# SebastienCoube/Improving-performances-of-MCMC-for-Nearest-Neighbor-Gaussian-Process-models-with-full-data-augmentat

Hardware: AMD Instinct MI355X
Metric: full-field Gibbs sweeps/sec at n=1e6, m=15; achieved HBM GB/s vs roofline (higher is better)
Workload: dtype f64

## Files before the change

### improving-performances-of-mcmc-for-nearest-neighbor-gaussian-process-models-with-full-data-augmentat_amd/csrc/capi.hip

```cpp
#include <hip/hip_runtime.h>
#include <rccl/rccl.h>

#include <algorithm>
#include <climits>
#include <cmath>
#include <cstdio>
#include <cstdlib>
#include <cstring>
#include <map>
#include <atomic>
#include <mutex>
#include <new>
#include <string>
#include <vector>

#include "../../include/nngp.h"
#include "graph_prep.h"
#include "kernels.h"
#include "rec_stream.h"

using namespace nngp;

struct ChainState {
  double* linv_d[2] = {nullptr, nullptr};
// ... 1656 lines not shown
  return NNGP_OK;
}

enum SweepPart { kPrologue = 1, kColours = 2, kEpilogue = 4, kAll = 7 };

static int enqueue_sweep_body(nngp_ctx* c, int n_sweeps, int mask, const double* z_dev, int parts = kAll) {
  const int n = c->n;
  SweepDev L = sweep_dev(c);
  FieldPtrs fp;
  for (int k = 0; k < kMaxChains; ++k) fp.p[k] = k < c->C ? c->ch[k].field_d : nullptr;
  if (parts & kPrologue) {
    HIPCHK(c, launch_field_to_slots_multi(c->st, c->n, c->slot_dpos_d, fp, c->scal_d, c->w_slot_d, c->C, mask));
    HIPCHK(c, launch_spmv_chains(c->st, c->linv_cur_d, c->nn_d, n, c->b, fp, c->scal_d, c->r_d, c->C, mask));
    if (!z_dev && c->engine == 0) HIPCHK(c, launch_normals_compact(c->st, L, mask, 0, n, c->zbuf_d));
  }
  if ((parts & kColours) && c->engine == 1) {
    TileLaunch a;
    a.n_sweeps = n_sweeps;
    a.chain_mask = mask;
    a.z_in = z_dev;
    a.variant = c->tvariant;
    if (c->tcs) {
      a.stagger = c->tstagger;
      HIPCHK(c, launch_sweep_tiles_cs(c->st, tile_dev(c), a, c->tl.max_rows, c->tl.NTK, c->tl.max_batches,
                                      c->tl.max_gslots));
    } else {
      HIPCHK(c, launch_sweep_tiles(c->st, tile_dev(c), a, c->tl.max_rows, c->tl.NTK, c->tl.max_batches,
                                    c->tl.max_gslots));
    }
    HIPCHK(c, hipMemcpyAsync(c->tmo_h, c->ctl_d + 2, sizeof(unsigned), hipMemcpyDeviceToHost, c->st));
  }
  if ((parts & kColours) && c->engine == 0) {
    const size_t zn = (size_t)n * c->C;
    for (int s = 0; s < n_sweeps; ++s) {
      for (int col = 0; col < c->lay.K; ++col) {
        ColorLaunch a;
        a.chunk0 = c->lay.color_chunk_ptr[col];
        a.nch = c->lay.color_chunk_ptr[col + 1] - a.chunk0;
        a.chain_mask = mask;
        a.sweep_local = s;
        a.z_cur = z_dev ? z_dev + (size_t)s * zn : c->zbuf_d + (size_t)(s & 1) * zn;
        a.z_next = (!z_dev && s + 1 < n_sweeps) ? c->zbuf_d + (size_t)((s + 1) & 1) * zn : nullptr;
        a.pairs = c->pairs_d + c->pair_ptr[col];
        a.npairs = c->pair_ptr[col + 1] - c->pair_ptr[col];
        a.n = n;
        HIPCHK(c, launch_sweep_color(c->st, L, a));
      }
    }
  }
  if (parts & kEpilogue)
    HIPCHK(c, launch_slots_to_field_multi(c->st, c->n, c->slot_dpos_d, fp, c->scal_d, c->w_slot_d, c->C, mask));
  return NNGP_OK;
}

static int graph_for(nngp_ctx* c, int n_sweeps, int mask, hipGraphExec_t* out, int parts = kAll) {
  const long long key = ((long long)n_sweeps << 12) | ((long long)parts << 8) | mask;
  auto it = c->graphs.find(key);
  if (it == c->graphs.end()) {
    hipGraph_t g;
    HIPCHK(c, hipStreamBeginCapture(c->st, hipStreamCaptureModeThreadLocal));
    int rc = enqueue_sweep_body(c, n_sweeps, mask, nullptr, parts);
    hipError_t e = hipStreamEndCapture(c->st, &g);
    if (rc) return rc;
    if (e != hipSuccess) return fail_hip(c, e, "hipStreamEndCapture");
    hipGraphExec_t ex;
// ... 1049 lines not shown
```

### improving-performances-of-mcmc-for-nearest-neighbor-gaussian-process-models-with-full-data-augmentat_amd/csrc/kernels.h

```cpp
#pragma once
#include <hip/hip_runtime.h>
#include <cstdint>
#include <vector>

namespace nngp {

constexpr int kWave = 64;
constexpr int kBlock = 256;
constexpr int kRedBlocks = 4096;

struct SweepScalars {
  double inv_s2;
  double inv_t2;
  double beta0;
  double dshift;
  uint64_t seed;
  uint64_t counter_base;
};

constexpr int kSweepRows = 16;
constexpr int kMaxChains = 4;

constexpr int kPkRowBits = 25;
constexpr int kPkPadRow = (1 << kPkRowBits) - 1;
// ... 155 lines not shown
  const double* const* b1;
  unsigned* ctl;
  unsigned long long* dbg;
  int K, C, T, n;
  int max_gslots;
  int probe = 0;
  int xw = 0;
};

struct TileLaunch {
  int n_sweeps;
  int chain_mask;
  const double* z_in;
  int stagger = 0;
  int variant = 0;
};

constexpr int tile_double_buffer(int C, int NT) { return C <= 2 ? 1 : 0; }
constexpr int tile_rmax(int C, int NT) { return 4096 / NT; }
constexpr int tile_rmax_cs(int NT) { return 2048 / NT; }
constexpr int tile_gmax(int NT) { return NT == 256 ? 4 : (NT == 512 ? 3 : 1); }
constexpr int kTileRanksMax = 16;
struct TileShard {
  int G = 1, Tl = 0, tile0 = 0, rank0 = 0;
  const TileDev* devs = nullptr;
  const unsigned* call = nullptr;
  double* gx[kTileRanksMax] = {};
};
hipError_t launch_sweep_tiles(hipStream_t st, const TileDev& D, const TileLaunch& a, int max_rows, int NT,
                              int max_batches, int max_gslots, const TileShard* sh = nullptr, int grid = 0,
// ... 47 lines not shown
```

### improving-performances-of-mcmc-for-nearest-neighbor-gaussian-process-models-with-full-data-augmentat_amd/csrc/tiles.hip

```cpp
#include "kernels.h"
#include "device_common.h"
#include "graph_prep.h"

namespace nngp {

constexpr uint32_t kTPad = kTilePadRow;
constexpr uint32_t kTStart = kCellStart, kTEnd = kCellEnd;
constexpr int kTExported = kSlotExported;
constexpr int kTSlots = kTileSlotsMax;
static_assert(kTileQShift == kTileRowBits && kTileQMask + 1 >= (uint32_t)kTSlots && kTileRowBits + 11 <= 30,
              "cell_pk fields: local row | slot << kTileQShift | start << 30 | end << 31");
constexpr int kTSpreadLds = 82 * 1024;


typedef unsigned int u32x4_t __attribute__((ext_vector_type(4)));
typedef unsigned int u32x2_t __attribute__((ext_vector_type(2)));

__device__ __forceinline__ uint32_t tile_lr(uint32_t pk) { return (pk & kTPad) ^ kTPad; }



__global__ void set_ptr_kernel(const double** dst, int k, const double* p) {
  if (threadIdx.x == 0) dst[k] = p;
}
// ... 121 lines not shown
}

template <int C, int NT, int RMAX>
__device__ __forceinline__ void tile_load_cells(const TileDev& D, const int4 B, TileBatchRegs<C, NT, RMAX>& b, int t) {
  b.R = B.y & 0xFFFF;
  const bool live = t < (B.y >> 16);
#pragma unroll
  for (int j = 0; j < RMAX; ++j) {
    if (j < b.R && live) {
      const long long e = B.x + (long long)j * NT + t;
      b.pk[j] = __builtin_nontemporal_load(D.cell_pk + e);
#pragma unroll
      for (int ch = 0; ch < C; ++ch) b.v[j][ch] = __builtin_nontemporal_load(D.cell_val + ch * D.n_cells + e);
    } else {
      b.pk[j] = 0u;
      if constexpr (NT == 64) {
#pragma unroll
        for (int ch = 0; ch < C; ++ch) b.v[j][ch] = 0.0;
      }
    }
  }
}

template <int C, int NT, int RMAX, int SH, int CS = C>
__device__ __forceinline__ void tile_load_batch(const TileDev& D, const int4 B, TileBatchRegs<C, NT, RMAX>& b, int t) {
  tile_load_items<C, NT, RMAX, SH, CS>(D, B, b, t);
  tile_load_cells<C, NT, RMAX>(D, B, b, t);
}

template <int C, int NT, int RMAX, int CS = C>
__device__ __forceinline__ void tile_prep_items(const TileDev& D, const TileLaunch& a, const double* sc_s,
                                                const unsigned long long* seed_s, int s,
                                                TileBatchRegs<C, NT, RMAX>& b, int t, int var = 0) {
#pragma unroll
// ... 5 lines not shown
      double z = 0.0;
      if (var & 2) z = 0.0;
      else if (a.z_in) z = a.z_in[((size_t)s * D.n + b.x0 + q) * CS + ch];
      else z = normal_loc(seed_s[2 * ch], seed_s[2 * ch + 1] + s, (uint32_t)b.loc[k]);
      const double a0 = (var & 4) ? 1.0 : b.a0[k], a1 = (var & 4) ? 0.5 : b.a1[k], wk = (var & 4) ? 0.0 : b.w[k];
      const double P = a0 * inv_s2 + (double)((var & 4) ? 1 : b.nobs[k]) * inv_t2;
      const double cR = inv_t2 * a1 + inv_s2 * (a0 * wk);
      const double rs = rsqrt_pos(P);
      b.a0[k] = cR;
      b.a1[k] = rs * rs;
      b.zs[k] = z * rs;
    }
  }
}

template <int C, int GMAX>
struct TileGhostRegs {
  int lr[GMAX], gx[GMAX];
  double gv[GMAX][C];
};

template <int C, int NT, int GMAX>
__device__ __forceinline__ void tile_load_ghosts(const TileDev& D, int gb, int g1, TileGhostRegs<C, GMAX>& g, int t) {
#pragma unroll
  for (int k = 0; k < GMAX; ++k) {
    const int e = gb + k * NT + t;
    g.lr[k] = -1;
    if (e < g1) {
      const long long raw = __builtin_nontemporal_load(reinterpret_cast<const long long*>(D.gcell) + e);
      g.lr[k] = (int)(raw & 0xFFFFFFFFll);
      g.gx[k] = (int)(raw >> 32);
#pragma unroll
      for (int ch = 0; ch < C; ++ch) g.gv[k][ch] = __builtin_nontemporal_load(D.gval + ch * D.n_gcells + e);
    }
  }
}

struct TileState;
template <int C, int GMAX>
__device__ __forceinline__ void tile_ghost_adds(TileState& S, const TileGhostRegs<C, GMAX>& gr);

struct TileState {
  double* r_s;
  double* acc_s;
  double* wsum;
  double* sc_s;
  unsigned long long* seed_s;
  double* dsh_s;
  int4* batch_s;
  int* bptr_s;
  int* gptr_s;
  int* gsp_s;
  int* bsp_s;
  double* gdw_s;
  int* wflag;
  unsigned* spin_s;
  int* pub_s;
  __amdgpu_buffer_rsrc_t gran;
  unsigned call;
  int gsl;
  unsigned* tmo;
  int G;
  bool timed_out;
  int T, t, lane, wv, K, nph, ph;
  uint32_t lrmax;
  unsigned long long tp[8], t_prev;
};

template <int C, int GMAX>
__device__ __forceinline__ void tile_ghost_adds(TileState& S, const TileGhostRegs<C, GMAX>& gr) {
  double rv[GMAX][C], dv[GMAX][C];
#pragma unroll
  for (int k = 0; k < GMAX; ++k) {
    const bool ok = gr.lr[k] >= 0;
    const int row = ok ? gr.lr[k] : 0, x = ok ? gr.gx[k] : 0;
#pragma unroll
    for (int ch = 0; ch < C; ++ch) {
      rv[k][ch] = S.r_s[row * C + ch];
      dv[k][ch] = S.gdw_s[x * C + ch];
    }
  }
#pragma unroll
  for (int k = 0; k < GMAX; ++k)
    if (gr.lr[k] >= 0)
#pragma unroll
      for (int ch = 0; ch < C; ++ch) S.r_s[gr.lr[k] * C + ch] = rv[k][ch] + gr.gv[k][ch] * dv[k][ch];
}

#define TSTAMP(S, k)                                                      \
  do {                                                                    \
    if (PROBE == 1) {                                                          \
      asm volatile("s_waitcnt vmcnt(0) lgkmcnt(0)" ::: "memory");         \
      const unsigned long long now_ = __builtin_amdgcn_s_memrealtime();   \
      if ((k) >= 0) (S).tp[(k) < 0 ? 0 : (k)] += now_ - (S).t_prev;       \
      (S).t_prev = now_;                                                  \
    }                                                                     \
  } while (0)

constexpr int kTimelinePhases = 512;
constexpr int kTimelineSlots = 16;
#define TLSTAMP(S, k)                                                                         \
// ... 4 lines not shown


template <int CTRL, int RM, bool BC, int C>
__device__ __forceinline__ void seg_scan_step(double (&v)[C], int& f) {
  double e[C];
#pragma unroll
  for (int ch = 0; ch < C; ++ch) e[ch] = dpp_f64<CTRL, RM, BC>(v[ch]);
  const int fe = __builtin_amdgcn_update_dpp(0, f, CTRL, RM, 0xF, BC);
  const double keep = f ? 0.0 : 1.0;
#pragma unroll
  for (int ch = 0; ch < C; ++ch) v[ch] = __builtin_fma(e[ch], keep, v[ch]);
  f |= fe;
}

constexpr int kOwnDrawBarriers = 3;
template <int C, int RMAX, int GRP, class TB>
__device__ __forceinline__ void tile_products(const TB& b, int R, const double* __restrict__ r_s,
                                              double* __restrict__ acc_s, uint32_t lrmax, double (&run)[C],
                                              int& cont_q, bool& seen_start) {
#pragma unroll
  for (int ch = 0; ch < C; ++ch) run[ch] = 0.0;
#pragma unroll
  for (int j0 = 0; j0 < RMAX; j0 += GRP) {
    if (j0 >= R) break;
    double rv[GRP][C];
#pragma unroll
    for (int jj = 0; jj < GRP; ++jj) {
      if (j0 + jj < RMAX) {
        const uint32_t lr = min(tile_lr(b.pk[j0 + jj]), lrmax);
#pragma unroll
        for (int ch = 0; ch < C; ++ch) rv[jj][ch] = r_s[lr * C + ch];
      }
    }
#pragma unroll
    for (int jj = 0; jj < GRP; ++jj) {
      const int j = j0 + jj;
      if (j < RMAX) {
        const uint32_t pk = b.pk[j];
        const bool st = (pk & kTStart) != 0;
        const double keep = st ? 0.0 : 1.0;
#pragma unroll
        for (int ch = 0; ch < C; ++ch) run[ch] = __builtin_fma(run[ch], keep, b.v[j][ch] * rv[jj][ch]);
        const int q = (int)((pk >> kTileQShift) & kTileQMask);
        if (pk & kTEnd) {
#pragma unroll
          for (int ch = 0; ch < C; ++ch) acc_s[q * C + ch] = run[ch];
// ... 15 lines not shown
  const int R = b.R, nit = b.ns * C;
  tile_cells_landed(b);
  double run[C];
  int cont_q = -1;
  bool seen_start = false;
#pragma unroll
  for (int ch = 0; ch < C; ++ch) run[ch] = 0.0;
#pragma unroll
  for (int j = 0; j < RMAX; ++j) {
    if (j < R) {
      const uint32_t pk = b.pk[j];
      const uint32_t lr = min(tile_lr(pk), S.lrmax);
      const bool st = (pk & kTStart) != 0;
      const double keep = st ? 0.0 : 1.0;
#pragma unroll
      for (int ch = 0; ch < C; ++ch) run[ch] = __builtin_fma(run[ch], keep, b.v[j][ch] * r_s[lr * C + ch]);
      const int q = (int)((pk >> kTileQShift) & kTileQMask);
      if (pk & kTEnd) {
#pragma unroll
        for (int ch = 0; ch < C; ++ch) acc_s[q * C + ch] = run[ch];
      }
      seen_start |= st;
      cont_q = ((pk & kTEnd) && !seen_start && cont_q < 0) ? q : cont_q;
    }
  }
  TSTAMP(S, 1);
  double v[C];
  int f = seen_start ? 1 : 0;
#pragma unroll
  for (int ch = 0; ch < C; ++ch) v[ch] = run[ch];
  seg_scan_step<0x111, 0xF, true, C>(v, f);
// ... 47 lines not shown
#pragma unroll
          for (int h = 0; h < kTileRanksMax; ++h)
            if (h < S.G && ((b.rm[k] >> h) & 1u))
              __builtin_amdgcn_raw_buffer_store_b128(
                  g, __builtin_amdgcn_make_buffer_rsrc(sh.gx[h], 0, 0x7FFFFFFF, 0x00020000), (int)(xu * 16), 0,
                  kGranAuxSys);
        }
      }
    }
  }
  __syncthreads();
  TSTAMP(S, 3);
  TLSTAMP(S, 1);
}

template <int C, int NT, int RMAX, int PROBE>
__device__ __forceinline__ void tile_own_scatter(TileState& S, const TileBatchRegs<C, NT, RMAX>& b, int R,
                                                 const double* acc_base = nullptr) {
  constexpr int GRP = RMAX < 4 ? RMAX : 4;
  double* r_s = S.r_s;
  const double* acc_s = acc_base ? acc_base : S.acc_s;
#pragma unroll
  for (int j0 = 0; j0 < RMAX; j0 += GRP) {
    if (j0 >= R) break;
    double rv[GRP][C], dv[GRP][C];
#pragma unroll
    for (int jj = 0; jj < GRP; ++jj) {
      const int j = j0 + jj;
      const uint32_t lr = tile_lr(b.pk[j]);
      const bool ok = j < R && lr != kTPad;
      const int row = ok ? (int)lr : 0, q = ok ? (int)((b.pk[j] >> kTileQShift) & kTileQMask) : 0;
#pragma unroll
      for (int ch = 0; ch < C; ++ch) {
        rv[jj][ch] = r_s[row * C + ch];
        dv[jj][ch] = acc_s[q * C + ch];
      }
    }
#pragma unroll
    for (int jj = 0; jj < GRP; ++jj) {
      const int j = j0 + jj;
      const uint32_t lr = tile_lr(b.pk[j]);
      if (j < R && lr != kTPad) {
#pragma unroll
        for (int ch = 0; ch < C; ++ch) r_s[lr * C + ch] = rv[jj][ch] + b.v[j][ch] * dv[jj][ch];
      }
    }
  }
  TSTAMP(S, 4);
}

template <int C, int NT, int RMAX>
__device__ __forceinline__ void tile_cells_landed(const TileBatchRegs<C, NT, RMAX>& b) {
#pragma unroll
  for (int j = 0; j < RMAX; ++j) {
    asm volatile("" ::"v"(b.pk[j]));
#pragma unroll
    for (int ch = 0; ch < C; ++ch) asm volatile("" ::"v"(b.v[j][ch]));
  }
}
// ... 197 lines not shown
    const int R = cur.R;
    if (bi + 1 == bend && more) tile_load_items<C, NT, RMAX, SH>(D, S.batch_s[S.bptr_s[cn]], cur, t);
    tile_own_scatter<C, NT, RMAX, PROBE>(S, cur, R);
  }
  if (more) {
    if (had_bnd) tile_load_cells<C, NT, RMAX>(D, S.batch_s[S.bptr_s[cn]], cur, t);
    else if (!had_int) tile_load_batch<C, NT, RMAX, SH>(D, S.batch_s[S.bptr_s[cn]], cur, t);
    tile_prep_items<C, NT, RMAX>(D, a, S.sc_s, S.seed_s, sn, cur, t);
  }
  __syncthreads();
  TLSTAMP(S, 3);
}

__device__ __forceinline__ void wave_lds_order() { asm volatile("s_waitcnt lgkmcnt(0)" ::: "memory"); }

template <int C, int RMAX, int PROBE, int SH>
__device__ __forceinline__ void tile_own_wl(const TileDev& D, const TileLaunch& a, const TileShard& sh, TileState& S,
                                            TileBatchRegs<C, 64, RMAX>& b, unsigned epoch, double* acc_w,
                                            bool first = false) {
  constexpr int IMAX = TileBatchRegs<C, 64, RMAX>::IMAX;
  const int lane = S.lane;
  const double* __restrict__ r_s = S.r_s;
  double* __restrict__ acc_s = acc_w;
  const int R = b.R, nit = b.ns * C;
  tile_cells_landed(b);
  double run[C];
  int cont_q = -1;
  bool seen_start = false;
  tile_products<C, RMAX, 4>(b, R, r_s, acc_s, S.lrmax, run, cont_q, seen_start);
  double v[C];
  int f = seen_start ? 1 : 0;
#pragma unroll
  for (int ch = 0; ch < C; ++ch) v[ch] = run[ch];
  seg_scan_step<0x111, 0xF, true, C>(v, f);
  seg_scan_step<0x112, 0xF, true, C>(v, f);
  seg_scan_step<0x114, 0xF, true, C>(v, f);
  seg_scan_step<0x118, 0xF, true, C>(v, f);
  seg_scan_step<0x142, 0xA, false, C>(v, f);
  seg_scan_step<0x143, 0xC, false, C>(v, f);
#pragma unroll
  for (int ch = 0; ch < C; ++ch) {
    const double up = dpp_f64<0x138, 0xF, true>(v[ch]);
    const double cp = lane ? up : 0.0;
    if (cont_q >= 0) acc_s[cont_q * C + ch] = acc_s[cont_q * C + ch] + cp;
// ... 22 lines not shown
          for (int h = 0; h < kTileRanksMax; ++h)
            if (h < S.G && ((b.rm[k] >> h) & 1u))
              __builtin_amdgcn_raw_buffer_store_b128(
                  g, __builtin_amdgcn_make_buffer_rsrc(sh.gx[h], 0, 0x7FFFFFFF, 0x00020000), (int)(xu * 16), 0,
                  kGranAuxSys);
        }
      }
    }
  }
  wave_lds_order();
  TLSTAMP(S, 1);
  if (PROBE == 2 && lane == 0 && S.ph < kTimelinePhases && S.wv < 7)
    D.dbg[((size_t)S.T * kTimelinePhases + S.ph) * kTimelineSlots + 9 + S.wv] = __builtin_amdgcn_s_memrealtime();
}

template <int C, int NT, int RMAX, int GMAX, int PROBE, int SH, int DB>
__device__ __forceinline__ void tile_phase_wl(const TileDev& D, const TileLaunch& a, const TileShard& sh,
                                              TileState& S, int ph, TileBatchRegs<C, 64, RMAX>& cur,
                                              TileBatchRegs<C, 64, RMAX>& nxt, TileGhostRegs<C, GMAX>& gr) {
  constexpr int W = NT / 64 - 1;
  const int K = S.K, t = S.t, lane = S.lane;
  const int s = ph / K, c = ph - s * K;
  const unsigned epoch = (unsigned)ph + 1;
  S.ph = ph;
  TLSTAMP(S, 0);
  const int phn = ph + 1;
  const int cn = phn % K, sn = phn / K;
  const bool has_next = phn < S.nph;
  const int bnext = S.bptr_s[cn] + S.wv;
  const bool more = has_next && bnext < S.bptr_s[cn + 1];
  const int bfirst = S.bptr_s[c] + S.wv, bend = S.bptr_s[c + 1];
  const int g0 = S.gptr_s[c], g1 = S.gptr_s[c + 1];
  double* acc_w = S.acc_s + S.wv * (kWaveSlotsMax * C);
  if (DB && more) tile_load_batch<C, 64, RMAX, SH>(D, S.batch_s[bnext], nxt, lane);
  for (int bi = bfirst; bi < bend; bi += W) {
    if (bi != bfirst) {
      tile_load_batch<C, 64, RMAX, SH>(D, S.batch_s[bi], cur, lane);
      tile_prep_items<C, 64, RMAX>(D, a, S.sc_s, S.seed_s, s, cur, lane);
    }
    tile_own_wl<C, RMAX, PROBE, SH>(D, a, sh, S, cur, epoch, acc_w, bi == bfirst);
    if (bi == bfirst && S.wv == 0 && lane == 0)
      __hip_atomic_store(S.pub_s, ph, __ATOMIC_RELAXED, __HIP_MEMORY_SCOPE_WORKGROUP);
    const int R = cur.R;
    if (bi + W >= bend) {
      if (!DB && more) tile_load_items<C, 64, RMAX, SH>(D, S.batch_s[bnext], nxt, lane);
      if (g1 > g0) tile_load_ghosts<C, NT, GMAX>(D, g0, g1, gr, t);
    }
    tile_own_scatter<C, 64, RMAX, PROBE>(S, cur, R, acc_w);
  }
  if (bfirst >= bend) {
    if (!DB && more) tile_load_items<C, 64, RMAX, SH>(D, S.batch_s[bnext], nxt, lane);
    if (g1 > g0) tile_load_ghosts<C, NT, GMAX>(D, g0, g1, gr, t);
  }
  TLSTAMP(S, 6);
  if (more) tile_prep_items<C, 64, RMAX>(D, a, S.sc_s, S.seed_s, sn, nxt, lane, PROBE == 2 ? a.variant : 0);
  if (!DB && more) tile_load_cells<C, 64, RMAX>(D, S.batch_s[bnext], nxt, lane);
  TLSTAMP(S, 4);
  __syncthreads();
  TLSTAMP(S, 2);
  for (int gb = g0; gb < g1; gb += NT * GMAX) {
    if (gb != g0) tile_load_ghosts<C, NT, GMAX>(D, gb, g1, gr, t);
    tile_ghost_adds<C, GMAX>(S, gr);
  }
  __syncthreads();
  TLSTAMP(S, 3);
}

template <int C, int NT, int RMAX, int GMAX, int PROBE, int SH>
__device__ __forceinline__ int tile_wlib_first(const TileState& S, int c) {
  const int fi = S.bptr_s[c] + S.wv, fb = S.bsp_s[c] + S.wv;
  return fi < S.bsp_s[c] ? fi : (fb < S.bptr_s[c + 1] ? fb : -1);
}

template <int C, int NT, int RMAX, int GMAX, int PROBE, int SH>
__device__ __forceinline__ void tile_phase_wlib(const TileDev& D, const TileLaunch& a, const TileShard& sh,
                                                TileState& S, int ph, TileBatchRegs<C, 64, RMAX>& cur,
                                                TileGhostRegs<C, GMAX>& gr) {
  constexpr int W = NT / 64 - 1;
  const int K = S.K, t = S.t, lane = S.lane;
  const int s = ph / K, c = ph - s * K;
  const unsigned epoch = (unsigned)ph + 1;
  S.ph = ph;
  TLSTAMP(S, 0);
  const int phn = ph + 1;
  const int cn = phn % K, sn = phn / K;
  const int nxt_b = phn < S.nph ? tile_wlib_first<C, NT, RMAX, GMAX, PROBE, SH>(S, cn) : -1;
  const int bsp = S.bsp_s[c], b1 = S.bptr_s[c + 1];
  const int ifirst = S.bptr_s[c] + S.wv, bfirst = bsp + S.wv;
  const bool hp = ph > 0;
  const int cp = hp ? (ph - 1) % K : 0;
  const int g0 = S.gptr_s[cp], g1 = hp ? S.gptr_s[cp + 1] : g0;
  double* acc_w = S.acc_s + S.wv * (kWaveSlotsMax * C);
  bool nx_items = false;
  for (int bi = ifirst; bi < bsp; bi += W) {
    if (bi != ifirst) {
      tile_load_batch<C, 64, RMAX, SH>(D, S.batch_s[bi], cur, lane);
      tile_prep_items<C, 64, RMAX>(D, a, S.sc_s, S.seed_s, s, cur, lane);
    }
    tile_own_wl<C, RMAX, PROBE, SH>(D, a, sh, S, cur, epoch, acc_w);
    const int R = cur.R;
    if (bi + W >= bsp) {
      if (bfirst < b1) {
        tile_load_items<C, 64, RMAX, SH>(D, S.batch_s[bfirst], cur, lane);
      } else if (nxt_b >= 0) {
        tile_load_items<C, 64, RMAX, SH>(D, S.batch_s[nxt_b], cur, lane);
        nx_items = true;
      }
      if (g1 > g0) tile_load_ghosts<C, NT, GMAX>(D, g0, g1, gr, t);
    }
    tile_own_scatter<C, 64, RMAX, PROBE>(S, cur, R, acc_w);
  }
  if (ifirst >= bsp) {
    if (g1 > g0) tile_load_ghosts<C, NT, GMAX>(D, g0, g1, gr, t);
  } else if (bfirst < b1) {
    tile_prep_items<C, 64, RMAX>(D, a, S.sc_s, S.seed_s, s, cur, lane);
    tile_load_cells<C, 64, RMAX>(D, S.batch_s[bfirst], cur, lane);
  }
  TLSTAMP(S, 6);
  __syncthreads();
  TLSTAMP(S, 4);
  for (int gb = g0; gb < g1; gb += NT * GMAX) {
    if (gb != g0) tile_load_ghosts<C, NT, GMAX>(D, gb, g1, gr, t);
    tile_ghost_adds<C, GMAX>(S, gr);
  }
  __syncthreads();
  TLSTAMP(S, 2);
  for (int bi = bfirst; bi < b1; bi += W) {
    if (bi != bfirst) {
      tile_load_batch<C, 64, RMAX, SH>(D, S.batch_s[bi], cur, lane);
      tile_prep_items<C, 64, RMAX>(D, a, S.sc_s, S.seed_s, s, cur, lane);
    }
    tile_own_wl<C, RMAX, PROBE, SH>(D, a, sh, S, cur, epoch, acc_w);
    const int R = cur.R;
    if (bi + W >= b1 && nxt_b >= 0) {
      tile_load_items<C, 64, RMAX, SH>(D, S.batch_s[nxt_b], cur, lane);
      nx_items = true;
    }
    tile_own_scatter<C, 64, RMAX, PROBE>(S, cur, R, acc_w);
  }
  if (nxt_b >= 0) {
    if (!nx_items) tile_load_items<C, 64, RMAX, SH>(D, S.batch_s[nxt_b], cur, lane);
    tile_prep_items<C, 64, RMAX>(D, a, S.sc_s, S.seed_s, sn, cur, lane);
    tile_load_cells<C, 64, RMAX>(D, S.batch_s[nxt_b], cur, lane);
  }
  __syncthreads();
  TLSTAMP(S, 3);
}


template <int C, int NT, int GMAX, int PROBE, int SH, int WL = 0, int LAG = 0>
__device__ __forceinline__ void tile_phase_xw(const TileDev& D, TileState& S, int ph, TileGhostRegs<C, GMAX>& gr) {
  constexpr int PB = 4;
  const int K = S.K, t = S.t, lane = S.lane;
  S.ph = ph;
  if (LAG && ph == 0) {
    __syncthreads();
    __syncthreads();
    __syncthreads();
    return;
  }
  const int phx = ph - LAG;
  const int c = phx % K;
  const unsigned epoch = (unsigned)phx + 1;
  const int bfirst = S.bptr_s[c], bend = S.bptr_s[c + 1];
  const int g0 = S.gptr_s[c], g1 = S.gptr_s[c + 1];
// ... 49 lines not shown
      }
      __builtin_amdgcn_s_sleep(1);
#pragma unroll
      for (int k = 0; k < PB; ++k)
        if ((pend >> k) & 1u) g[k] = __builtin_amdgcn_raw_buffer_load_b128(S.gran, off[k], 0, aux);
    }
  }
  if (PROBE == 2 && lane == 0 && S.ph < kTimelinePhases) {
    D.dbg[((size_t)S.T * kTimelinePhases + S.ph) * kTimelineSlots + 7] = __builtin_amdgcn_s_memrealtime();
    D.dbg[((size_t)S.T * kTimelinePhases + S.ph) * kTimelineSlots + 5] = *S.spin_s;
    *S.spin_s = 0;
  }
  __syncthreads();
  for (int gb = g0; gb < g1; gb += NT * GMAX) {
    if (gb != g0) tile_load_ghosts<C, NT, GMAX>(D, gb, g1, gr, t);
    tile_ghost_adds<C, GMAX>(S, gr);
  }
  __syncthreads();
  if (LAG && ph < S.nph) __syncthreads();
}

template <int C, int NT, int NTC, int RMAX, int GMAX, int DB, int PROBE, int SH>
__device__ __forceinline__ void tile_phase_cells(const TileDev& D, const TileLaunch& a, const TileShard& sh,
                                                 TileState& S, int ph, TileBatchRegs<C, NTC, RMAX>& cur,
                                                 TileBatchRegs<C, NTC, RMAX>& nxt, TileGhostRegs<C, GMAX>& gr) {
  const int K = S.K, t = S.t;
  const int s = ph / K, c = ph - s * K;
  const unsigned epoch = (unsigned)ph + 1;
  S.ph = ph;
  TLSTAMP(S, 0);
  const int phn = ph + 1;
// ... 28 lines not shown
  }
  TLSTAMP(S, 6);
  if (more) tile_prep_items<C, NTC, RMAX>(D, a, S.sc_s, S.seed_s, sn, nxt, t);
  if (!DB && more) tile_load_cells<C, NTC, RMAX>(D, S.batch_s[S.bptr_s[cn]], nxt, t);
  TLSTAMP(S, 4);
  __syncthreads();
  TLSTAMP(S, 2);
  for (int gb = g0; gb < g1; gb += NT * GMAX) {
    if (gb != g0) tile_load_ghosts<C, NT, GMAX>(D, gb, g1, gr, t);
    tile_ghost_adds<C, GMAX>(S, gr);
  }
  __syncthreads();
  TLSTAMP(S, 3);
}

template <int C, int NT, int RMAX, int GMAX, int DB, int PROBE, int SH, int RG, int IB, int CS, int XW = 0>
__device__ __forceinline__ void sweep_tiles_body(const TileDev& D0, TileLaunch a, const TileShard& sh) {
  static_assert(!XW || ((!RG || XW == 2) && (!IB || XW == 2) && CS == C),
                "exchange-wave tiles: joint chains; split layouts and r in global memory only with wave-local batches");
  constexpr int NTC = XW ? NT - 64 : NT;
  using BR = TileBatchRegs<C, NTC, RMAX>;
  constexpr int NW = NT / 64;
  extern __shared__ __attribute__((aligned(16))) double smem[];
  int Tg = SH ? sh.tile0 + (int)blockIdx.x : (int)blockIdx.x;
  const int rk = SH ? Tg / sh.Tl : 0;
  TileDev D = SH ? sh.devs[rk - sh.rank0] : D0;
  int ch0 = 0;
  if constexpr (CS != C) {
    static_assert(C == 1 && !SH && !RG && !IB && !PROBE, "chain-split: one chain per workgroup, single GPU");
    ch0 = Tg / D.T;
    Tg -= ch0 * D.T;
    D.cell_val += (size_t)ch0 * D.n_cells;
    D.gval += (size_t)ch0 * D.n_gcells;
    D.dr += ch0;
    D.w_slot += ch0;
// ... 4 lines not shown
    a.chain_mask >>= ch0;
    if (a.z_in) a.z_in += ch0;
  }
  TileState S;
  S.G = SH ? sh.G : 1;
  S.T = Tg; S.t = threadIdx.x; S.lane = S.t & 63; S.wv = S.t >> 6; S.K = D.K;
  S.nph = a.n_sweeps * D.K;
  S.timed_out = false;
  for (int k = 0; k < 8; ++k) S.tp[k] = 0;
  S.t_prev = 0;
  const int T = S.T, t = S.t, K = D.K;
  const int row0 = D.erow_ptr[T], nrows = D.erow_ptr[T + 1] - row0;
  S.lrmax = nrows > 0 ? (uint32_t)(nrows - 1) : 0u;
  const int b_lo = D.batch_ptr[T * K], nbt = D.batch_ptr[T * K + K] - b_lo;
  S.r_s = RG ? D.rg + (size_t)row0 * C : smem;
  S.acc_s = RG ? smem : smem + ((nrows * C + 1) / 2) * 2;
  S.wsum = S.acc_s + kAccSlots * C;
  S.sc_s = S.wsum + NW * C;
  S.seed_s = reinterpret_cast<unsigned long long*>(S.sc_s + 2 * C);
  S.dsh_s = reinterpret_cast<double*>(S.seed_s + 2 * C);
  S.gdw_s = S.dsh_s + C;
  S.batch_s = reinterpret_cast<int4*>(S.gdw_s + ((D.max_gslots * C + 1) / 2) * 2);
  S.bptr_s = reinterpret_cast<int*>(S.batch_s + nbt);
  S.gptr_s = S.bptr_s + K + 1;
  S.gsp_s = S.gptr_s + K + 1;
  S.bsp_s = S.gsp_s + K + 1;
  S.wflag = S.bsp_s + K + 1;
  S.spin_s = reinterpret_cast<unsigned*>(S.wflag + NW);
  if (PROBE == 2 && t == 0) *S.spin_s = 0;
  S.pub_s = reinterpret_cast<int*>(S.spin_s + 1);
  if (t == 0) *S.pub_s = -1;
  TSTAMP(S, -1);
  double dsh[C];
#pragma unroll
  for (int ch = 0; ch < C; ++ch) dsh[ch] = D.scal[ch].dshift;
  for (int lr = t; lr < nrows; lr += NT) {
    const int row = D.erow[row0 + lr];
    const size_t g = (size_t)row * CS;
#pragma unroll
    for (int ch = 0; ch < C; ++ch) {
      const double v = D.r[g + ch];
      S.r_s[lr * C + ch] = dsh[ch] != 0.0 ? __builtin_fma(-dsh[ch], D.b1[ch][row], v) : v;
    }
  }
  for (int i = t; i < nbt; i += NT) S.batch_s[i] = D.batch[b_lo + i];
  for (int i = t; i <= K; i += NT) {
    S.bptr_s[i] = D.batch_ptr[T * K + i] - b_lo;
    S.gptr_s[i] = D.gptr[T * K + i];
    S.gsp_s[i] = D.gslot_ptr[T * K + i];
    if (IB) S.bsp_s[i] = i < K ? D.batch_split[T * K + i] - b_lo : 0;
  }
  if (t < C) {
    S.dsh_s[t] = D.scal[t].dshift;
    S.sc_s[2 * t] = D.scal[t].inv_s2;
    S.sc_s[2 * t + 1] = D.scal[t].inv_t2;
    S.seed_s[2 * t] = D.scal[t].seed;
    S.seed_s[2 * t + 1] = D.scal[t].counter_base;
// ... 4 lines not shown
  S.gran = __builtin_amdgcn_make_buffer_rsrc(SH ? sh.gx[rk] : D.dwx, 0, 0x7FFFFFFF, 0x00020000);
  __syncthreads();
  bool shifted = false;
#pragma unroll
  for (int ch = 0; ch < C; ++ch) shifted |= dsh[ch] != 0.0;
  if (shifted && nbt > 0) {
    const int x0 = S.batch_s[0].w, x1 = S.batch_s[nbt - 1].w + S.batch_s[nbt - 1].z;
    for (int u = t; u < (x1 - x0) * C; u += NT) D.w_slot[tile_xu<C, CS>(x0, u)] -= S.dsh_s[u % C];
    __syncthreads();
  }
  if constexpr (XW) {
    if (S.wv == NW - 1) {
      TileGhostRegs<C, GMAX> GX;
      __syncthreads();
      if constexpr (IB) {
        for (int ph = 0; ph <= S.nph; ++ph) tile_phase_xw<C, NT, GMAX, PROBE, SH, 1, 1>(D, S, ph, GX);
      } else {
        for (int ph = 0; ph < S.nph; ++ph) tile_phase_xw<C, NT, GMAX, PROBE, SH, XW == 2>(D, S, ph, GX);
      }
    } else if constexpr (XW == 2 && IB) {
      TileBatchRegs<C, 64, RMAX> A;
      TileGhostRegs<C, GMAX> GA;
      const int f0 = S.nph > 0 ? tile_wlib_first<C, NT, RMAX, GMAX, PROBE, SH>(S, 0) : -1;
      if (f0 >= 0) {
        tile_load_batch<C, 64, RMAX, SH>(D, S.batch_s[f0], A, S.lane);
        tile_prep_items<C, 64, RMAX>(D, a, S.sc_s, S.seed_s, 0, A, S.lane);
      }
      __syncthreads();
      for (int ph = 0; ph < S.nph; ++ph) tile_phase_wlib<C, NT, RMAX, GMAX, PROBE, SH>(D, a, sh, S, ph, A, GA);
      const int cp = S.nph > 0 ? (S.nph - 1) % K : 0;
      const int g0 = S.gptr_s[cp], g1 = S.nph > 0 ? S.gptr_s[cp + 1] : g0;
      if (g1 > g0) tile_load_ghosts<C, NT, GMAX>(D, g0, g1, GA, t);
      if (S.nph > 0) {
        __syncthreads();
        for (int gb = g0; gb < g1; gb += NT * GMAX) {
          if (gb != g0) tile_load_ghosts<C, NT, GMAX>(D, gb, g1, GA, t);
          tile_ghost_adds<C, GMAX>(S, GA);
        }
        __syncthreads();
      } else {
        __syncthreads();
        __syncthreads();
      }
    } else if constexpr (XW == 2) {
      TileBatchRegs<C, 64, RMAX> A, B;
      TileGhostRegs<C, GMAX> GA;
      if (S.nph > 0 && S.bptr_s[0] + S.wv < S.bptr_s[1]) {
        tile_load_batch<C, 64, RMAX, SH>(D, S.batch_s[S.bptr_s[0] + S.wv], A, S.lane);
        tile_prep_items<C, 64, RMAX>(D, a, S.sc_s, S.seed_s, 0, A, S.lane);
      }
      __syncthreads();
      if (DB) {
        for (int ph = 0; ph < S.nph; ph += 2) {
          tile_phase_wl<C, NT, RMAX, GMAX, PROBE, SH, DB>(D, a, sh, S, ph, A, B, GA);
          if (ph + 1 < S.nph) tile_phase_wl<C, NT, RMAX, GMAX, PROBE, SH, DB>(D, a, sh, S, ph + 1, B, A, GA);
        }
      } else {
        for (int ph = 0; ph < S.nph; ++ph) tile_phase_wl<C, NT, RMAX, GMAX, PROBE, SH, DB>(D, a, sh, S, ph, A, A, GA);
      }
    } else {
      BR A, B;
      TileGhostRegs<C, GMAX> GA;
      if (S.nph > 0 && S.bptr_s[0] < S.bptr_s[1]) {
        tile_load_batch<C, NTC, RMAX, SH>(D, S.batch_s[S.bptr_s[0]], A, t);
        tile_prep_items<C, NTC, RMAX>(D, a, S.sc_s, S.seed_s, 0, A, t);
      }
      __syncthreads();
      if (DB) {
        for (int ph = 0; ph < S.nph; ph += 2) {
          tile_phase_cells<C, NT, NTC, RMAX, GMAX, DB, PROBE, SH>(D, a, sh, S, ph, A, B, GA);
          if (ph + 1 < S.nph) tile_phase_cells<C, NT, NTC, RMAX, GMAX, DB, PROBE, SH>(D, a, sh, S, ph + 1, B, A, GA);
        }
      } else {
// ... 15 lines not shown
    const unsigned long long t0 = __builtin_amdgcn_s_memrealtime();
    while (__builtin_amdgcn_s_memrealtime() - t0 < (unsigned long long)ch0 * (unsigned)a.stagger) __builtin_amdgcn_s_sleep(4);
  }
  if (DB) {
    for (int ph = 0; ph < S.nph; ph += 2) {
      tile_phase<C, NT, RMAX, GMAX, DB, PROBE, SH, CS>(D, a, sh, S, ph, A, B, GA, GB);
      if (ph + 1 < S.nph) tile_phase<C, NT, RMAX, GMAX, DB, PROBE, SH, CS>(D, a, sh, S, ph + 1, B, A, GB, GA);
    }
  } else if (IB) {
    for (int ph = 0; ph < S.nph; ++ph) tile_phase_ib<C, NT, RMAX, GMAX, PROBE, SH>(D, a, sh, S, ph, A, GA);
  } else {
    for (int ph = 0; ph < S.nph; ++ph) tile_phase<C, NT, RMAX, GMAX, DB, PROBE, SH, CS>(D, a, sh, S, ph, A, A, GA, GA);
  }
  }
  __syncthreads();
  for (int lr = t; lr < nrows; lr += NT) {
    double* rg = const_cast<double*>(D.r) + (size_t)D.erow[row0 + lr] * CS;
#pragma unroll
    for (int ch = 0; ch < C; ++ch) rg[ch] = S.r_s[lr * C + ch];
  }
  if (PROBE == 1 && t == 0) {
    unsigned long long* o = D.dbg + (size_t)T * 8;
    for (int k = 0; k < 8; ++k) o[k] = S.tp[k];
  }
}

template <int C, int NT, int RMAX, int GMAX, int DB, int PROBE, int SH, int RG, int IB, int XW>
__global__ __launch_bounds__(NT) void sweep_tiles_kernel(TileDev D0, TileLaunch a, TileShard sh) {
  sweep_tiles_body<C, NT, RMAX, GMAX, DB, PROBE, SH, RG, IB, C, XW>(D0, a, sh);
}

template <int CS, int NT, int RMAX, int GMAX>
__global__ __launch_bounds__(NT) __attribute__((amdgpu_waves_per_eu(CS * NT / 256, CS * NT / 256)))
void sweep_tiles_cs_kernel(TileDev D0, TileLaunch a) {
// ... 244 lines not shown
```

Measured before the change: 14780.

## Fuse slot-to-field epilogue into tile sweep kernel; chain-major LDS residuals

When the tile engine runs a full sweep unsharded, each tile block now writes its slots back to the field arrays (adding beta0) at the end of the sweep kernel, and the separate slots_to_field launch is skipped. This removes one kernel launch and a pass over the slot data. For C=3 exchange-wave layouts the shared-memory residual array becomes chain-major to reduce LDS bank conflicts. The residual write-back and the new tail loop are unrolled by four to add memory-level parallelism. The risks are a tail imbalance inside the sweep kernel, and that the fused epilogue assumes each tile's batch slot range covers exactly the slots it owns.

```diff
diff --git a/improving-performances-of-mcmc-for-nearest-neighbor-gaussian-process-models-with-full-data-augmentat_amd/csrc/capi.hip b/improving-performances-of-mcmc-for-nearest-neighbor-gaussian-process-models-with-full-data-augmentat_amd/csrc/capi.hip
--- a/improving-performances-of-mcmc-for-nearest-neighbor-gaussian-process-models-with-full-data-augmentat_amd/csrc/capi.hip
+++ b/improving-performances-of-mcmc-for-nearest-neighbor-gaussian-process-models-with-full-data-augmentat_amd/csrc/capi.hip
@@ -1694,12 +1694,21 @@
     HIPCHK(c, launch_spmv_chains(c->st, c->linv_cur_d, c->nn_d, n, c->b, fp, c->scal_d, c->r_d, c->C, mask));
     if (!z_dev && c->engine == 0) HIPCHK(c, launch_normals_compact(c->st, L, mask, 0, n, c->zbuf_d));
   }
+#ifdef NNGP_NO_FUSED_FIELD
+  const bool fused = false;
+#else
+  const bool fused = (parts & kColours) && (parts & kEpilogue) && c->engine == 1 && !c->shard && n_sweeps > 0;
+#endif
   if ((parts & kColours) && c->engine == 1) {
     TileLaunch a;
     a.n_sweeps = n_sweeps;
     a.chain_mask = mask;
     a.z_in = z_dev;
     a.variant = c->tvariant;
+    if (fused) {
+      a.slot_dpos = c->slot_dpos_d;
+      a.field = fp;
+    }
     if (c->tcs) {
       a.stagger = c->tstagger;
       HIPCHK(c, launch_sweep_tiles_cs(c->st, tile_dev(c), a, c->tl.max_rows, c->tl.NTK, c->tl.max_batches,
@@ -1728,7 +1737,7 @@
       }
     }
   }
-  if (parts & kEpilogue)
+  if ((parts & kEpilogue) && !fused)
     HIPCHK(c, launch_slots_to_field_multi(c->st, c->n, c->slot_dpos_d, fp, c->scal_d, c->w_slot_d, c->C, mask));
   return NNGP_OK;
 }
diff --git a/improving-performances-of-mcmc-for-nearest-neighbor-gaussian-process-models-with-full-data-augmentat_amd/csrc/kernels.h b/improving-performances-of-mcmc-for-nearest-neighbor-gaussian-process-models-with-full-data-augmentat_amd/csrc/kernels.h
--- a/improving-performances-of-mcmc-for-nearest-neighbor-gaussian-process-models-with-full-data-augmentat_amd/csrc/kernels.h
+++ b/improving-performances-of-mcmc-for-nearest-neighbor-gaussian-process-models-with-full-data-augmentat_amd/csrc/kernels.h
@@ -193,6 +193,8 @@
   const double* z_in;
   int stagger = 0;
   int variant = 0;
+  const int* slot_dpos = nullptr;
+  FieldPtrs field = {};
 };
 
 constexpr int tile_double_buffer(int C, int NT) { return C <= 2 ? 1 : 0; }
diff --git a/improving-performances-of-mcmc-for-nearest-neighbor-gaussian-process-models-with-full-data-augmentat_amd/csrc/tiles.hip b/improving-performances-of-mcmc-for-nearest-neighbor-gaussian-process-models-with-full-data-augmentat_amd/csrc/tiles.hip
--- a/improving-performances-of-mcmc-for-nearest-neighbor-gaussian-process-models-with-full-data-augmentat_amd/csrc/tiles.hip
+++ b/improving-performances-of-mcmc-for-nearest-neighbor-gaussian-process-models-with-full-data-augmentat_amd/csrc/tiles.hip
@@ -159,10 +159,8 @@
       for (int ch = 0; ch < C; ++ch) b.v[j][ch] = __builtin_nontemporal_load(D.cell_val + ch * D.n_cells + e);
     } else {
       b.pk[j] = 0u;
-      if constexpr (NT == 64) {
-#pragma unroll
-        for (int ch = 0; ch < C; ++ch) b.v[j][ch] = 0.0;
-      }
+#pragma unroll
+      for (int ch = 0; ch < C; ++ch) b.v[j][ch] = 0.0;
     }
   }
 }
@@ -198,6 +196,18 @@
   }
 }
 
+constexpr int tile_r_chain_major(int C, int RG, int SH, int XW) {
+#ifdef NNGP_TILE_R_INTERLEAVED
+  return 0;
+#else
+  return C == 3 && !RG && !SH && XW == 2;
+#endif
+}
+template <int C, int CM>
+__device__ __forceinline__ int tile_r_index(int lr, int ch, int RS) {
+  return CM ? ch * RS + lr : lr * C + ch;
+}
+
 template <int C, int GMAX>
 struct TileGhostRegs {
   int lr[GMAX], gx[GMAX];
@@ -221,11 +231,12 @@
 }
 
 struct TileState;
-template <int C, int GMAX>
+template <int C, int GMAX, int CM = 0>
 __device__ __forceinline__ void tile_ghost_adds(TileState& S, const TileGhostRegs<C, GMAX>& gr);
 
 struct TileState {
   double* r_s;
+  int RS;
   double* acc_s;
   double* wsum;
   double* sc_s;
@@ -251,7 +262,7 @@
   unsigned long long tp[8], t_prev;
 };
 
-template <int C, int GMAX>
+template <int C, int GMAX, int CM>
 __device__ __forceinline__ void tile_ghost_adds(TileState& S, const TileGhostRegs<C, GMAX>& gr) {
   double rv[GMAX][C], dv[GMAX][C];
 #pragma unroll
@@ -260,7 +271,7 @@
     const int row = ok ? gr.lr[k] : 0, x = ok ? gr.gx[k] : 0;
 #pragma unroll
     for (int ch = 0; ch < C; ++ch) {
-      rv[k][ch] = S.r_s[row * C + ch];
+      rv[k][ch] = S.r_s[tile_r_index<C, CM>(row, ch, S.RS)];
       dv[k][ch] = S.gdw_s[x * C + ch];
     }
   }
@@ -268,7 +279,7 @@
   for (int k = 0; k < GMAX; ++k)
     if (gr.lr[k] >= 0)
 #pragma unroll
-      for (int ch = 0; ch < C; ++ch) S.r_s[gr.lr[k] * C + ch] = rv[k][ch] + gr.gv[k][ch] * dv[k][ch];
+      for (int ch = 0; ch < C; ++ch) S.r_s[tile_r_index<C, CM>(gr.lr[k], ch, S.RS)] = rv[k][ch] + gr.gv[k][ch] * dv[k][ch];
 }
 
 #define TSTAMP(S, k)                                                      \
@@ -303,8 +314,8 @@
 }
 
 constexpr int kOwnDrawBarriers = 3;
-template <int C, int RMAX, int GRP, class TB>
-__device__ __forceinline__ void tile_products(const TB& b, int R, const double* __restrict__ r_s,
+template <int C, int RMAX, int GRP, int CM, class TB>
+__device__ __forceinline__ void tile_products(const TB& b, int R, const double* __restrict__ r_s, int RS,
                                               double* __restrict__ acc_s, uint32_t lrmax, double (&run)[C],
                                               int& cont_q, bool& seen_start) {
 #pragma unroll
@@ -318,7 +329,7 @@
       if (j0 + jj < RMAX) {
         const uint32_t lr = min(tile_lr(b.pk[j0 + jj]), lrmax);
 #pragma unroll
-        for (int ch = 0; ch < C; ++ch) rv[jj][ch] = r_s[lr * C + ch];
+        for (int ch = 0; ch < C; ++ch) rv[jj][ch] = r_s[tile_r_index<C, CM>((int)lr, ch, RS)];
       }
     }
 #pragma unroll
@@ -364,7 +375,7 @@
       const bool st = (pk & kTStart) != 0;
       const double keep = st ? 0.0 : 1.0;
 #pragma unroll
-      for (int ch = 0; ch < C; ++ch) run[ch] = __builtin_fma(run[ch], keep, b.v[j][ch] * r_s[lr * C + ch]);
+      for (int ch = 0; ch < C; ++ch) run[ch] = __builtin_fma(run[ch], keep, b.v[j][ch] * r_s[tile_r_index<C, 0>((int)lr, ch, 0)]);
       const int q = (int)((pk >> kTileQShift) & kTileQMask);
       if (pk & kTEnd) {
 #pragma unroll
@@ -442,7 +453,7 @@
   TLSTAMP(S, 1);
 }
 
-template <int C, int NT, int RMAX, int PROBE>
+template <int C, int NT, int RMAX, int PROBE, int CM = 0>
 __device__ __forceinline__ void tile_own_scatter(TileState& S, const TileBatchRegs<C, NT, RMAX>& b, int R,
                                                  const double* acc_base = nullptr) {
   constexpr int GRP = RMAX < 4 ? RMAX : 4;
@@ -460,7 +471,7 @@
       const int row = ok ? (int)lr : 0, q = ok ? (int)((b.pk[j] >> kTileQShift) & kTileQMask) : 0;
 #pragma unroll
       for (int ch = 0; ch < C; ++ch) {
-        rv[jj][ch] = r_s[row * C + ch];
+        rv[jj][ch] = r_s[tile_r_index<C, CM>(row, ch, S.RS)];
         dv[jj][ch] = acc_s[q * C + ch];
       }
     }
@@ -470,7 +481,7 @@
       const uint32_t lr = tile_lr(b.pk[j]);
       if (j < R && lr != kTPad) {
 #pragma unroll
-        for (int ch = 0; ch < C; ++ch) r_s[lr * C + ch] = rv[jj][ch] + b.v[j][ch] * dv[jj][ch];
+        for (int ch = 0; ch < C; ++ch) r_s[tile_r_index<C, CM>((int)lr, ch, S.RS)] = rv[jj][ch] + b.v[j][ch] * dv[jj][ch];
       }
     }
   }
@@ -698,7 +709,7 @@
 
 __device__ __forceinline__ void wave_lds_order() { asm volatile("s_waitcnt lgkmcnt(0)" ::: "memory"); }
 
-template <int C, int RMAX, int PROBE, int SH>
+template <int C, int RMAX, int PROBE, int SH, int CM>
 __device__ __forceinline__ void tile_own_wl(const TileDev& D, const TileLaunch& a, const TileShard& sh, TileState& S,
                                             TileBatchRegs<C, 64, RMAX>& b, unsigned epoch, double* acc_w,
                                             bool first = false) {
@@ -711,7 +722,7 @@
   double run[C];
   int cont_q = -1;
   bool seen_start = false;
-  tile_products<C, RMAX, 4>(b, R, r_s, acc_s, S.lrmax, run, cont_q, seen_start);
+  tile_products<C, RMAX, 4, CM>(b, R, r_s, S.RS, acc_s, S.lrmax, run, cont_q, seen_start);
   double v[C];
   int f = seen_start ? 1 : 0;
 #pragma unroll
@@ -764,7 +775,7 @@
     D.dbg[((size_t)S.T * kTimelinePhases + S.ph) * kTimelineSlots + 9 + S.wv] = __builtin_amdgcn_s_memrealtime();
 }
 
-template <int C, int NT, int RMAX, int GMAX, int PROBE, int SH, int DB>
+template <int C, int NT, int RMAX, int GMAX, int PROBE, int SH, int DB, int CM>
 __device__ __forceinline__ void tile_phase_wl(const TileDev& D, const TileLaunch& a, const TileShard& sh,
                                               TileState& S, int ph, TileBatchRegs<C, 64, RMAX>& cur,
                                               TileBatchRegs<C, 64, RMAX>& nxt, TileGhostRegs<C, GMAX>& gr) {
@@ -788,7 +799,7 @@
       tile_load_batch<C, 64, RMAX, SH>(D, S.batch_s[bi], cur, lane);
       tile_prep_items<C, 64, RMAX>(D, a, S.sc_s, S.seed_s, s, cur, lane);
     }
-    tile_own_wl<C, RMAX, PROBE, SH>(D, a, sh, S, cur, epoch, acc_w, bi == bfirst);
+    tile_own_wl<C, RMAX, PROBE, SH, CM>(D, a, sh, S, cur, epoch, acc_w, bi == bfirst);
     if (bi == bfirst && S.wv == 0 && lane == 0)
       __hip_atomic_store(S.pub_s, ph, __ATOMIC_RELAXED, __HIP_MEMORY_SCOPE_WORKGROUP);
     const int R = cur.R;
@@ -796,7 +807,7 @@
       if (!DB && more) tile_load_items<C, 64, RMAX, SH>(D, S.batch_s[bnext], nxt, lane);
       if (g1 > g0) tile_load_ghosts<C, NT, GMAX>(D, g0, g1, gr, t);
     }
-    tile_own_scatter<C, 64, RMAX, PROBE>(S, cur, R, acc_w);
+    tile_own_scatter<C, 64, RMAX, PROBE, CM>(S, cur, R, acc_w);
   }
   if (bfirst >= bend) {
     if (!DB && more) tile_load_items<C, 64, RMAX, SH>(D, S.batch_s[bnext], nxt, lane);
@@ -810,7 +821,7 @@
   TLSTAMP(S, 2);
   for (int gb = g0; gb < g1; gb += NT * GMAX) {
     if (gb != g0) tile_load_ghosts<C, NT, GMAX>(D, gb, g1, gr, t);
-    tile_ghost_adds<C, GMAX>(S, gr);
+    tile_ghost_adds<C, GMAX, CM>(S, gr);
   }
   __syncthreads();
   TLSTAMP(S, 3);
@@ -822,7 +833,7 @@
   return fi < S.bsp_s[c] ? fi : (fb < S.bptr_s[c + 1] ? fb : -1);
 }
 
-template <int C, int NT, int RMAX, int GMAX, int PROBE, int SH>
+template <int C, int NT, int RMAX, int GMAX, int PROBE, int SH, int CM>
 __device__ __forceinline__ void tile_phase_wlib(const TileDev& D, const TileLaunch& a, const TileShard& sh,
                                                 TileState& S, int ph, TileBatchRegs<C, 64, RMAX>& cur,
                                                 TileGhostRegs<C, GMAX>& gr) {
@@ -847,7 +858,7 @@
       tile_load_batch<C, 64, RMAX, SH>(D, S.batch_s[bi], cur, lane);
       tile_prep_items<C, 64, RMAX>(D, a, S.sc_s, S.seed_s, s, cur, lane);
     }
-    tile_own_wl<C, RMAX, PROBE, SH>(D, a, sh, S, cur, epoch, acc_w);
+    tile_own_wl<C, RMAX, PROBE, SH, CM>(D, a, sh, S, cur, epoch, acc_w);
     const int R = cur.R;
     if (bi + W >= bsp) {
       if (bfirst < b1) {
@@ -858,7 +869,7 @@
       }
       if (g1 > g0) tile_load_ghosts<C, NT, GMAX>(D, g0, g1, gr, t);
     }
-    tile_own_scatter<C, 64, RMAX, PROBE>(S, cur, R, acc_w);
+    tile_own_scatter<C, 64, RMAX, PROBE, CM>(S, cur, R, acc_w);
   }
   if (ifirst >= bsp) {
     if (g1 > g0) tile_load_ghosts<C, NT, GMAX>(D, g0, g1, gr, t);
@@ -871,7 +882,7 @@
   TLSTAMP(S, 4);
   for (int gb = g0; gb < g1; gb += NT * GMAX) {
     if (gb != g0) tile_load_ghosts<C, NT, GMAX>(D, gb, g1, gr, t);
-    tile_ghost_adds<C, GMAX>(S, gr);
+    tile_ghost_adds<C, GMAX, CM>(S, gr);
   }
   __syncthreads();
   TLSTAMP(S, 2);
@@ -880,13 +891,13 @@
       tile_load_batch<C, 64, RMAX, SH>(D, S.batch_s[bi], cur, lane);
       tile_prep_items<C, 64, RMAX>(D, a, S.sc_s, S.seed_s, s, cur, lane);
     }
-    tile_own_wl<C, RMAX, PROBE, SH>(D, a, sh, S, cur, epoch, acc_w);
+    tile_own_wl<C, RMAX, PROBE, SH, CM>(D, a, sh, S, cur, epoch, acc_w);
     const int R = cur.R;
     if (bi + W >= b1 && nxt_b >= 0) {
       tile_load_items<C, 64, RMAX, SH>(D, S.batch_s[nxt_b], cur, lane);
       nx_items = true;
     }
-    tile_own_scatter<C, 64, RMAX, PROBE>(S, cur, R, acc_w);
+    tile_own_scatter<C, 64, RMAX, PROBE, CM>(S, cur, R, acc_w);
   }
   if (nxt_b >= 0) {
     if (!nx_items) tile_load_items<C, 64, RMAX, SH>(D, S.batch_s[nxt_b], cur, lane);
@@ -898,7 +909,7 @@
 }
 
 
-template <int C, int NT, int GMAX, int PROBE, int SH, int WL = 0, int LAG = 0>
+template <int C, int NT, int GMAX, int PROBE, int SH, int WL = 0, int LAG = 0, int CM = 0>
 __device__ __forceinline__ void tile_phase_xw(const TileDev& D, TileState& S, int ph, TileGhostRegs<C, GMAX>& gr) {
   constexpr int PB = 4;
   const int K = S.K, t = S.t, lane = S.lane;
@@ -978,7 +989,7 @@
   __syncthreads();
   for (int gb = g0; gb < g1; gb += NT * GMAX) {
     if (gb != g0) tile_load_ghosts<C, NT, GMAX>(D, gb, g1, gr, t);
-    tile_ghost_adds<C, GMAX>(S, gr);
+    tile_ghost_adds<C, GMAX, CM>(S, gr);
   }
   __syncthreads();
   if (LAG && ph < S.nph) __syncthreads();
@@ -1037,11 +1048,13 @@
   TLSTAMP(S, 3);
 }
 
+constexpr int kTailU = 4;
 template <int C, int NT, int RMAX, int GMAX, int DB, int PROBE, int SH, int RG, int IB, int CS, int XW = 0>
 __device__ __forceinline__ void sweep_tiles_body(const TileDev& D0, TileLaunch a, const TileShard& sh) {
   static_assert(!XW || ((!RG || XW == 2) && (!IB || XW == 2) && CS == C),
                 "exchange-wave tiles: joint chains; split layouts and r in global memory only with wave-local batches");
   constexpr int NTC = XW ? NT - 64 : NT;
+  constexpr int CM = CS == C ? tile_r_chain_major(C, RG, SH, XW) : 0;
   using BR = TileBatchRegs<C, NTC, RMAX>;
   constexpr int NW = NT / 64;
   extern __shared__ __attribute__((aligned(16))) double smem[];
@@ -1076,6 +1089,7 @@
   S.lrmax = nrows > 0 ? (uint32_t)(nrows - 1) : 0u;
   const int b_lo = D.batch_ptr[T * K], nbt = D.batch_ptr[T * K + K] - b_lo;
   S.r_s = RG ? D.rg + (size_t)row0 * C : smem;
+  S.RS = nrows;
   S.acc_s = RG ? smem : smem + ((nrows * C + 1) / 2) * 2;
   S.wsum = S.acc_s + kAccSlots * C;
   S.sc_s = S.wsum + NW * C;
@@ -1102,7 +1116,7 @@
 #pragma unroll
     for (int ch = 0; ch < C; ++ch) {
       const double v = D.r[g + ch];
-      S.r_s[lr * C + ch] = dsh[ch] != 0.0 ? __builtin_fma(-dsh[ch], D.b1[ch][row], v) : v;
+      S.r_s[tile_r_index<C, CM>(lr, ch, S.RS)] = dsh[ch] != 0.0 ? __builtin_fma(-dsh[ch], D.b1[ch][row], v) : v;
     }
   }
   for (int i = t; i < nbt; i += NT) S.batch_s[i] = D.batch[b_lo + i];
@@ -1137,9 +1151,9 @@
       TileGhostRegs<C, GMAX> GX;
       __syncthreads();
       if constexpr (IB) {
-        for (int ph = 0; ph <= S.nph; ++ph) tile_phase_xw<C, NT, GMAX, PROBE, SH, 1, 1>(D, S, ph, GX);
+        for (int ph = 0; ph <= S.nph; ++ph) tile_phase_xw<C, NT, GMAX, PROBE, SH, 1, 1, CM>(D, S, ph, GX);
       } else {
-        for (int ph = 0; ph < S.nph; ++ph) tile_phase_xw<C, NT, GMAX, PROBE, SH, XW == 2>(D, S, ph, GX);
+        for (int ph = 0; ph < S.nph; ++ph) tile_phase_xw<C, NT, GMAX, PROBE, SH, XW == 2, 0, CM>(D, S, ph, GX);
       }
     } else if constexpr (XW == 2 && IB) {
       TileBatchRegs<C, 64, RMAX> A;
@@ -1150,7 +1164,7 @@
         tile_prep_items<C, 64, RMAX>(D, a, S.sc_s, S.seed_s, 0, A, S.lane);
       }
       __syncthreads();
-      for (int ph = 0; ph < S.nph; ++ph) tile_phase_wlib<C, NT, RMAX, GMAX, PROBE, SH>(D, a, sh, S, ph, A, GA);
+      for (int ph = 0; ph < S.nph; ++ph) tile_phase_wlib<C, NT, RMAX, GMAX, PROBE, SH, CM>(D, a, sh, S, ph, A, GA);
       const int cp = S.nph > 0 ? (S.nph - 1) % K : 0;
       const int g0 = S.gptr_s[cp], g1 = S.nph > 0 ? S.gptr_s[cp + 1] : g0;
       if (g1 > g0) tile_load_ghosts<C, NT, GMAX>(D, g0, g1, GA, t);
@@ -1158,7 +1172,7 @@
         __syncthreads();
         for (int gb = g0; gb < g1; gb += NT * GMAX) {
           if (gb != g0) tile_load_ghosts<C, NT, GMAX>(D, gb, g1, GA, t);
-          tile_ghost_adds<C, GMAX>(S, GA);
+          tile_ghost_adds<C, GMAX, CM>(S, GA);
         }
         __syncthreads();
       } else {
@@ -1175,11 +1189,11 @@
       __syncthreads();
       if (DB) {
         for (int ph = 0; ph < S.nph; ph += 2) {
-          tile_phase_wl<C, NT, RMAX, GMAX, PROBE, SH, DB>(D, a, sh, S, ph, A, B, GA);
-          if (ph + 1 < S.nph) tile_phase_wl<C, NT, RMAX, GMAX, PROBE, SH, DB>(D, a, sh, S, ph + 1, B, A, GA);
+          tile_phase_wl<C, NT, RMAX, GMAX, PROBE, SH, DB, CM>(D, a, sh, S, ph, A, B, GA);
+          if (ph + 1 < S.nph) tile_phase_wl<C, NT, RMAX, GMAX, PROBE, SH, DB, CM>(D, a, sh, S, ph + 1, B, A, GA);
         }
       } else {
-        for (int ph = 0; ph < S.nph; ++ph) tile_phase_wl<C, NT, RMAX, GMAX, PROBE, SH, DB>(D, a, sh, S, ph, A, A, GA);
+        for (int ph = 0; ph < S.nph; ++ph) tile_phase_wl<C, NT, RMAX, GMAX, PROBE, SH, DB, CM>(D, a, sh, S, ph, A, A, GA);
       }
     } else {
       BR A, B;
@@ -1225,10 +1239,50 @@
   }
   }
   __syncthreads();
-  for (int lr = t; lr < nrows; lr += NT) {
-    double* rg = const_cast<double*>(D.r) + (size_t)D.erow[row0 + lr] * CS;
-#pragma unroll
-    for (int ch = 0; ch < C; ++ch) rg[ch] = S.r_s[lr * C + ch];
+  if (a.slot_dpos && nbt > 0) {
+    double* fld[C];
+    double b0[C];
+#pragma unroll
+    for (int ch = 0; ch < C; ++ch) {
+      if constexpr (CS == C) {
+        fld[ch] = a.field.p[ch];
+      } else {
+        static_assert(kMaxChains == 4, "the chain's field pointer is picked by selects");
+        fld[ch] = ch0 == 0 ? a.field.p[0] : ch0 == 1 ? a.field.p[1] : ch0 == 2 ? a.field.p[2] : a.field.p[3];
+      }
+      b0[ch] = D.scal[ch].beta0;
+    }
+    const int x0 = S.batch_s[0].w, x1 = S.batch_s[nbt - 1].w + S.batch_s[nbt - 1].z;
+    for (int x = x0 + t; x < x1; x += NT * kTailU) {
+      int d[kTailU];
+      double w[kTailU][C];
+#pragma unroll
+      for (int u = 0; u < kTailU; ++u) {
+        const int xs = x + u * NT;
+        d[u] = xs < x1 ? a.slot_dpos[xs] : -1;
+#pragma unroll
+        for (int ch = 0; ch < C; ++ch)
+          w[u][ch] = (xs < x1 && ((a.chain_mask >> ch) & 1)) ? D.w_slot[(size_t)xs * CS + ch] : 0.0;
+      }
+#pragma unroll
+      for (int u = 0; u < kTailU; ++u)
+        if (d[u] >= 0)
+#pragma unroll
+          for (int ch = 0; ch < C; ++ch)
+            if ((a.chain_mask >> ch) & 1) fld[ch][d[u]] = w[u][ch] + b0[ch];
+    }
+  }
+  for (int lr = t; lr < nrows; lr += NT * kTailU) {
+    int row[kTailU];
+#pragma unroll
+    for (int u = 0; u < kTailU; ++u) row[u] = lr + u * NT < nrows ? D.erow[row0 + lr + u * NT] : -1;
+#pragma unroll
+    for (int u = 0; u < kTailU; ++u) {
+      if (row[u] < 0) continue;
+      double* rg = const_cast<double*>(D.r) + (size_t)row[u] * CS;
+#pragma unroll
+      for (int ch = 0; ch < C; ++ch) rg[ch] = S.r_s[tile_r_index<C, CM>(lr + u * NT, ch, S.RS)];
+    }
   }
   if (PROBE == 1 && t == 0) {
     unsigned long long* o = D.dbg + (size_t)T * 8;
```

After: 15000, median of 6. 1.5% higher.
